# r-barnes/richdem

Hardware: AMD Instinct MI355X
Metric: Mcells/s Priority-Flood fill, 40k x 40k f32 DEM (higher is better)
Workload: dtype f32; 1 GPU; 40000x40000 float32 fractal value-noise DEM G(seed=3), FillDepressions<D8>, HBM-resident; cells=1600000000, basins=10332798, boruvka_rounds=9, pair_records=39443188, jump_passes=1, parallelism=1 GPU

## Files before the change

### richdem_amd/csrc/fill.hip

```cpp
#include "common.hpp"

#include <algorithm>
#include <cstdlib>
#include <vector>

struct rdgpu_fill_shard;

namespace rdgpu {

constexpr int TW = 64;
constexpr int TH = 32;
constexpr int LW = TW + 2;
constexpr int LH = TH + 2;
constexpr int NTHR = 256;
constexpr uint32_t OUTP = 0xFFFFFFFFu;
constexpr uint32_t CLOSED = 0x80000000u;
constexpr uint32_t NO_TID = 0xFFFFFFFFu;

static thread_local rdgpu_fill_stats g_stats;

constexpr int DW = 64, DH = 64, DLW = DW + 2, DLH = DH + 2;
constexpr uint32_t LAB_PEND = 0x80000000u;
constexpr uint16_t LTERM_BASE = 0xF000u;

// ... 2115 lines not shown
  const uint32_t n = st * rcap + i;
  const uint32_t c = cur[curN[n] & ~CLOSED] & ~CLOSED;
  nodeW[n] = c == B ? NO_TID : tid[c];
}

template <class T, int TOPO>
__global__ __launch_bounds__(NTHR) void k_shard_edges16(const T *__restrict__ z, const uint16_t *__restrict__ lab16,
                                                        const uint32_t *__restrict__ tile_base, uint32_t dtx,
                                                        const uint32_t *__restrict__ nodeW, const uint32_t *__restrict__ lvl,
                                                        int w, int h, unsigned long long *hkeys, uint32_t *hvals, uint32_t hmask,
                                                        uint32_t *overflow, uint32_t tilesX, uint32_t ntiles) {
  __shared__ uint32_t sl[ELH * ELW];
  __shared__ uint32_t sw[ELH * ELW];
  const uint32_t t = xcd_tile(blockIdx.x, ntiles);
  if (t >= ntiles) return;
  const int x0 = (int)(t % tilesX) * EW, y0 = (int)(t / tilesX) * EH;
  constexpr int IPT = (ELH * ELW + NTHR - 1) / NTHR;
  uint32_t nv[IPT], kv[IPT];
  bool ok[IPT];
#pragma unroll
  for (int r = 0; r < IPT; r++) {
    const int i = threadIdx.x + r * NTHR;
    const int ly = i / ELW, lx = i - ly * ELW;
    const int gx = x0 - 1 + lx, gy = y0 + ly;
    ok[r] = i < ELH * ELW && gx >= 0 && gx < w && gy < h;
    const int cx = ok[r] ? gx : 0, cy = ok[r] ? gy : 0;
    const size_t g = (size_t)cy * w + cx;
    nv[r] = tile_base[(uint32_t)(cy / DH) * dtx + (uint32_t)(cx / DW)] + lab16[g];
    kv[r] = Key32<T>::to(z[g]);
  }
  uint32_t wv[IPT], av[IPT];
#pragma unroll
  for (int r = 0; r < IPT; r++) {
    wv[r] = nodeW[nv[r]];
    av[r] = lvl[nv[r]];
  }
#pragma unroll
  for (int r = 0; r < IPT; r++) {
    const int i = threadIdx.x + r * NTHR;
    if (i < ELH * ELW) {
      sl[i] = ok[r] ? wv[r] : E_INVALID;
      sw[i] = av[r] > kv[r] ? av[r] : kv[r];
    }
  }
  __syncthreads();
  const int lx = threadIdx.x & (EW - 1), ly0 = threadIdx.x >> 6;
#pragma unroll 2
  for (int j = 0; j < EH / 4; j++) {
    const int ly = ly0 + 4 * j;
    const int o = ly * ELW + lx + 1;
    const uint32_t la = sl[o];
    if (la == E_INVALID) continue;
    const uint32_t wa = sw[o];
#pragma unroll
    for (int k = 0; k < 4; k++) {
      if (TOPO == 4 && (k == 1 || k == 3)) continue;
      const int q = o + (k == 0 ? 1 : k == 1 ? ELW - 1 : k == 2 ? ELW : ELW + 1);
      const uint32_t lb = sl[q];
      if (lb == la || lb == E_INVALID) continue;
      const uint32_t wb = sw[q];
      const uint32_t pass = wa > wb ? wa : wb;
      const uint32_t lo = la < lb ? la : lb, hi = la < lb ? lb : la;
      const unsigned long long key = (((unsigned long long)lo << 32) | hi) + 1ull;
      uint32_t slot = (uint32_t)((key * 0x9E3779B97F4A7C15ull) >> 32) & hmask;
      for (uint32_t probe = 0;; probe++) {
        if (probe > hmask) { *overflow = 1; break; }
        unsigned long long cur_k = __hip_atomic_load(&hkeys[slot], __ATOMIC_RELAXED, __HIP_MEMORY_SCOPE_AGENT);
        if (cur_k == 0) cur_k = atomicCAS(&hkeys[slot], 0ull, key);
        if (cur_k == 0 || cur_k == key) {
          if (__hip_atomic_load(&hvals[slot], __ATOMIC_RELAXED, __HIP_MEMORY_SCOPE_AGENT) > pass) atomicMin(&hvals[slot], pass);
          break;
        }
        slot = (slot + 1) & hmask;
      }
    }
  }
}

__global__ __launch_bounds__(NTHR) void k_node_levels(const uint32_t *__restrict__ curN, const uint32_t *__restrict__ acc,
                                                      const unsigned long long *__restrict__ counters, uint32_t rcap,
                                                      uint32_t *lvl) {
  const uint32_t st = blockIdx.y, i = blockIdx.x * NTHR + threadIdx.x;
  if (i >= (uint32_t)(counters[st * FSTRIDE] >> 32)) return;
  const uint32_t n = st * rcap + i;
  lvl[n] = acc[curN[n] & ~CLOSED];
}

template <class T, bool VEC>
__global__ __launch_bounds__(NTHR) void k_finalize16(T *z, const uint16_t *__restrict__ lab16, const uint32_t *__restrict__ lvl,
                                                     const uint32_t *__restrict__ tile_base, const uint32_t *__restrict__ tile_count,
                                                     int w, int h, uint32_t tilesX, uint32_t ntiles,
                                                     const uint8_t *__restrict__ skip = nullptr,
                                                     const uint32_t *__restrict__ tlist = nullptr,
                                                     const uint32_t *__restrict__ curN = nullptr,
                                                     const uint32_t *__restrict__ acc = nullptr) {
  __shared__ uint32_t sl[DH * DW];
  const uint32_t t = tlist ? tlist[blockIdx.x] : xcd_tile(blockIdx.x, ntiles);
  if (t >= ntiles) return;
  if (skip && skip[t]) return;
  const int x0 = (int)(t % tilesX) * DW, y0 = (int)(t / tilesX) * DH;
  const int qx = threadIdx.x & 15, ry = threadIdx.x >> 4;
  const int gx = x0 + 4 * qx;
  Quad<T> zqs[DH / 16];
  Quad<uint16_t> lqs[DH / 16];
#pragma unroll
  for (int r = 0; r < DH / 16; r++) {
    const int gy = y0 + ry + 16 * r;
    const bool in = gx < w && gy < h;
    const size_t g = in ? (size_t)gy * w + gx : 0;
    zqs[r] = load_quad<T, VEC>(z + (g - (in ? gx : 0)), in ? gx : 0, w, T());
    lqs[r] = load_quad<uint16_t, VEC>(lab16 + (g - (in ? gx : 0)), in ? gx : 0, w, (uint16_t)0);
  }
  const uint32_t base = tile_base[t], cnt = tile_count[t];
  if (curN) {
    for (uint32_t i = threadIdx.x; i < cnt; i += NTHR) sl[i] = acc[curN[base + i] & ~CLOSED];
  } else {
    for (uint32_t i = threadIdx.x; i < cnt; i += NTHR) sl[i] = lvl[base + i];
  }
  __syncthreads();
#pragma unroll
  for (int r = 0; r < DH / 16; r++) {
    const int gy = y0 + ry + 16 * r;
    if (gx >= w || gy >= h) continue;
    const size_t g = (size_t)gy * w + gx;
    Quad<T> zq = zqs[r];
    const Quad<uint16_t> lq = lqs[r];
    bool any = false;
#pragma unroll
    for (int e = 0; e < 4; e++) {
      if (gx + e >= w) continue;
      const uint32_t L = sl[lq.v[e] & (uint16_t)(DW * DH - 1)];
      if (L > Key32<T>::to(zq.v[e])) { zq.v[e] = Key32<T>::from(L); any = true; }
    }
    if (any) {
      if (VEC) {
        struct alignas(4 * sizeof(T)) AQ { T v[4]; };
        AQ a;
#pragma unroll
        for (int e = 0; e < 4; e++) a.v[e] = zq.v[e];
        *reinterpret_cast<AQ *>(z + g) = a;
      } else {
#pragma unroll
        for (int e = 0; e < 4; e++)
          if (gx + e < w) z[g + e] = zq.v[e];
      }
    }
  }
}

constexpr int NT_CAP = 1024;
static_assert(NT_CAP * 4 <= TW * TH * 2, "the node table lives in the boundary list's storage");
static_assert(TW == DW && DH % TH == 0, "a scan tile lies inside one descent tile");
constexpr uint32_t NO_TILE = 0xFFFFFFFFu;
constexpr int RING = 2 * LW + 2 * TH;

__device__ __forceinline__ void pair_spill_local(const EdgeOut &eo, unsigned long long *best, uint32_t seg, uint32_t *seg_fill,
                                                 uint32_t lo, uint32_t hi, uint32_t key) {
  const unsigned long long cl = ((unsigned long long)key << 32) | hi, ch = ((unsigned long long)key << 32) | lo;
  if (!(lo & CLOSED) && cl < best[lo]) atomicMin(&best[lo], cl);
  if (!(hi & CLOSED) && ch < best[hi]) atomicMin(&best[hi], ch);
  const uint32_t g = atomicAdd(seg_fill, 1u);
  if (g < eo.seglimit) {
    const size_t i = (size_t)seg * eo.segcap + g;
    eo.a[i] = lo; eo.b[i] = hi; eo.k[i] = key;
  } else {
    *eo.overflow = 1;
  }
}

template <class T, int TOPO, bool VEC>
__global__ __launch_bounds__(NTHR) void k_pairs16(const T *__restrict__ z, const uint16_t *__restrict__ lab16,
                                                  const uint32_t *__restrict__ curN, unsigned long long *best,
                                                  int w, int h, uint32_t B, uint32_t tilesX,
                                                  const uint32_t *__restrict__ tiles_in, uint32_t nwork,
                                                  EdgeOut eo,
                                                  const uint32_t *__restrict__ tile_base,
                                                  const uint32_t *__restrict__ tile_count, uint32_t dtx,
                                                  const uint8_t *__restrict__ skip,
                                                  const uint32_t *__restrict__ edgeK, const uint16_t *__restrict__ edgeS) {
  __shared__ __attribute__((aligned(8))) uint32_t sk[LH * LW];
  __shared__ uint32_t sc[LH * LW];
  __shared__ __attribute__((aligned(4))) uint16_t list[TW * TH];
  uint32_t *const ntab = reinterpret_cast<uint32_t *>(list);
  __shared__ unsigned long long pt_pair[PT_SLOTS];
  __shared__ uint32_t pt_key[PT_SLOTS];
  __shared__ uint32_t nlist, pt_n, pt_base, seg_fill;
  uint32_t *const tab_id = sk;
  unsigned long long *const tab_val = reinterpret_cast<unsigned long long *>(sk + SC_SLOTS);

  const uint32_t xcd = blockIdx.x & 7u, kstep = gridDim.x >> 3, per = (nwork + 7u) / 8u;
  const uint32_t seg = blockIdx.x;
  uint32_t it = blockIdx.x >> 3;
  auto next_tile = [&](uint32_t &i) -> uint32_t {
    while (i < per) {
      const uint32_t wi = xcd * per + i;
      if (wi >= nwork) break;
      const uint32_t t = tiles_in ? tiles_in[wi] : wi;
      if (!skip) return t;
      const int x0 = (int)(t % tilesX) * TW, y0 = (int)(t / tilesX) * TH;
      if (!skip[(uint32_t)(y0 / DH) * dtx + (uint32_t)(x0 / DW)]) return t;
      i += kstep;
    }
    i = per;
    return NO_TILE;
  };
  if (threadIdx.x == 0) seg_fill = 0;

  Quad<T> zq[2];
  Quad<uint16_t> lq[2];
  T rz = T();
  uint32_t rl = 0, rtb = 0, rc = 0, tbC = 0, cnt = 0, rkey = 0;
  uint32_t nt[NT_CAP / NTHR];
  auto ring_y = [](int tid) { const int rk = min(tid, RING - 1); return rk < LW ? 0 : rk < 2 * LW ? LH - 1 : (rk - 2 * LW < TH ? rk - 2 * LW + 1 : rk - 2 * LW - TH + 1); };
  auto ring_x = [](int tid) { const int rk = min(tid, RING - 1); return rk < LW ? rk : rk < 2 * LW ? rk - LW : (rk - 2 * LW < TH ? 0 : LW - 1); };

  auto load_a = [&](uint32_t t, int tid) {
    const int x0 = (int)(t % tilesX) * TW, y0 = (int)(t / tilesX) * TH;
    const uint32_t dC = (uint32_t)(y0 / DH) * dtx + (uint32_t)(x0 / DW);
    tbC = tile_base[dC];
    cnt = tile_count[dC];
    {
      const int rx = ring_x(tid), ry = ring_y(tid);
      const int gx = min(max(x0 - 1 + rx, 0), w - 1), gy = min(max(y0 - 1 + ry, 0), h - 1);
      const bool col = edgeK && ry >= 1 && ry <= TH && tid < RING;
      const uint32_t dtn = (uint32_t)(gy / DH) * dtx + (uint32_t)(gx / DW);
      const size_t e = ((size_t)dtn * 2 + (rx == 0 ? 1 : 0)) * DH + (uint32_t)(gy % DH);
      const size_t g = col ? (size_t)y0 * w + x0 : (size_t)gy * w + gx;
      rtb = tile_base[dtn];
      rl = col ? (uint32_t)edgeS[e] : (uint32_t)lab16[g];
      rkey = col ? edgeK[e] : 0u;
      rz = z[g];
    }
    const size_t tile0 = (size_t)y0 * w + x0;
    const char *zt = reinterpret_cast<const char *>(z + tile0), *lt = reinterpret_cast<const char *>(lab16 + tile0);
#pragma unroll
    for (int r = 0; r < 2; r++) {
      const int i = tid + r * NTHR;
      const int ly = i / (TW / 4), q = i - ly * (TW / 4);
      const int gx = x0 + 4 * q, gy = y0 + ly;
      const bool ok = gy < h && gx < w;
      if (VEC) {
        const uint32_t cell = ok ? (uint32_t)ly * (uint32_t)w + 4u * (uint32_t)q : 0u;
        struct alignas(4 * sizeof(T)) AZ { T v[4]; };
        struct alignas(8) AL { uint16_t v[4]; };
        const AL a = *reinterpret_cast<const AL *>(lt + cell * (uint32_t)sizeof(uint16_t));
        const AZ b = *reinterpret_cast<const AZ *>(zt + cell * (uint32_t)sizeof(T));
#pragma unroll
        for (int e = 0; e < 4; e++) { lq[r].v[e] = a.v[e]; zq[r].v[e] = b.v[e]; }
      } else {
        const size_t row = ok ? (size_t)gy * w : 0;
        lq[r] = load_quad<uint16_t, false>(lab16 + row, ok ? gx : 0, w, (uint16_t)0);
        zq[r] = load_quad<T, false>(z + row, ok ? gx : 0, w, T());
        if (!ok)
#pragma unroll
          for (int e = 0; e < 4; e++) lq[r].v[e] = 0;
      }
    }
  };
  auto load_b = [&](int tid) {
    const uint32_t nn = (cnt <= (uint32_t)NT_CAP && cnt) ? cnt : 1u;
#pragma unroll
    for (int k = 0; k < NT_CAP / NTHR; k++) {
      const uint32_t idx = (uint32_t)tid + k * NTHR;
      nt[k] = curN[tbC + min(idx, nn - 1u)];
    }
    rc = curN[rtb + rl];
  };

  uint32_t t = next_tile(it);
  if (t == NO_TILE) return;
  load_a(t, (int)threadIdx.x);
  load_b((int)threadIdx.x);
  constexpr int ROWS = TH / 4;
  for (;;) {
    int tid = (int)threadIdx.x;
    asm volatile("" : "+v"(tid));
    const int lx = tid & (TW - 1), band = __builtin_amdgcn_readfirstlane(tid >> 6), lane = tid & 63;
    const int rly = ring_y(tid), rlx = ring_x(tid);
    const bool isring = tid < RING;
    const int x0 = (int)(t % tilesX) * TW, y0 = (int)(t / tilesX) * TH;
    const bool tabled = cnt <= (uint32_t)NT_CAP;
#pragma unroll
    for (int k = 0; k < NT_CAP / NTHR; k++) ntab[tid + k * NTHR] = nt[k];
    pt_pair[tid] = ~0ull;
    pt_key[tid] = 0xFFFFFFFFu;
    static_assert(PT_SLOTS == NTHR, "one slot per thread");
    if (tid == 0) { nlist = 0; pt_n = 0; }
    __syncthreads();
    {
      uint32_t cq[2][4];
      if (tabled) {
#pragma unroll
        for (int r = 0; r < 2; r++)
#pragma unroll
          for (int e = 0; e < 4; e++) cq[r][e] = ntab[lq[r].v[e]];
      } else {
#pragma unroll
        for (int r = 0; r < 2; r++)
#pragma unroll
          for (int e = 0; e < 4; e++) cq[r][e] = curN[tbC + (uint32_t)lq[r].v[e]];
      }
      if (x0 + TW <= w && y0 + TH <= h) {
#pragma unroll
        for (int r = 0; r < 2; r++) {
          const int i = tid + r * NTHR;
          const int ly = i / (TW / 4), q = i - ly * (TW / 4);
          const int o = (ly + 1) * LW + 1 + 4 * q;
#pragma unroll
          for (int e = 0; e < 4; e++) {
            sk[o + e] = Key32<T>::to(zq[r].v[e]);
            sc[o + e] = cq[r][e];
          }
        }
      } else {
#pragma unroll
        for (int r = 0; r < 2; r++) {
          const int i = tid + r * NTHR;
          const int ly = i / (TW / 4), q = i - ly * (TW / 4);
          const int gx = x0 + 4 * q, gy = y0 + ly;
          const int o = (ly + 1) * LW + 1 + 4 * q;
#pragma unroll
          for (int e = 0; e < 4; e++) {
            const bool in = gy < h && gx + e < w;
            sk[o + e] = in ? Key32<T>::to(zq[r].v[e]) : 0u;
            sc[o + e] = in ? cq[r][e] : (B | CLOSED);
          }
        }
      }
      if (isring) {
        const int gx = x0 - 1 + rlx, gy = y0 - 1 + rly;
        const bool ok = gx >= 0 && gx < w && gy >= 0 && gy < h;
        const bool col = edgeK && rly >= 1 && rly <= TH;
        sk[rly * LW + rlx] = ok ? (col ? rkey : Key32<T>::to(rz)) : 0u;
        sc[rly * LW + rlx] = ok ? rc : (B | CLOSED);
      }
    }
    it += kstep;
    const uint32_t tn = next_tile(it);
    const uint32_t tl = tn != NO_TILE ? tn : t;
    load_a(tl, tid);
    __syncthreads();
    const int gxl = x0 + lx;
    const int yb = band * ROWS;
    {
      uint32_t c1[3], c2[3];
      {
        const int o = (yb + 1) * LW + lx;
#pragma unroll
        for (int e = 0; e < 3; e++) c1[e] = sc[o + e];
      }
      unsigned long long bal[ROWS];
      bool bnd[ROWS];
      const int rows_in = min(h - y0 - yb, ROWS);
      const bool colin = gxl < w;
#pragma unroll
      for (int j = 0; j < ROWS; j++) {
        const int ly = yb + j;
        {
          const int o = (ly + 2) * LW + lx;
#pragma unroll
          for (int e = 0; e < 3; e++) c2[e] = sc[o + e];
        }
        const uint32_t C = c1[1];
        uint32_t df = (c1[2] ^ C) | (c2[1] ^ C);
        if (TOPO == 8) df |= (c2[0] ^ C) | (c2[2] ^ C);
        bnd[j] = df != 0 && colin && j < rows_in;
        bal[j] = __builtin_amdgcn_ballot_w64(bnd[j]);
#pragma unroll
        for (int e = 0; e < 3; e++) c1[e] = c2[e];
      }
      uint32_t total = 0;
#pragma unroll
      for (int j = 0; j < ROWS; j++) total += (uint32_t)__popcll(bal[j]);
      if (total) {
        uint32_t base = 0;
        if (lane == 0) base = atomicAdd(&nlist, total);
        base = __shfl(base, 0, 64);
#pragma unroll
        for (int j = 0; j < ROWS; j++) {
          if (bnd[j])
            list[base + __builtin_amdgcn_mbcnt_hi((uint32_t)(bal[j] >> 32), __builtin_amdgcn_mbcnt_lo((uint32_t)bal[j], 0u))] =
                (uint16_t)((yb + j + 1) * LW + lx + 1);
          base += (uint32_t)__popcll(bal[j]);
        }
      }
    }
    __syncthreads();
    load_b(tid);
    const uint32_t nl = nlist;
    constexpr int NF = TOPO == 8 ? 4 : 2;
    const int foff[4] = {1, TOPO == 8 ? LW + 1 : LW, LW, LW - 1};
    for (uint32_t i = tid; i < nl; i += NTHR) {
      const int o = list[i];
      const uint32_t C = sc[o], kc = sk[o];
      uint32_t nD[NF], nH[NF];
#pragma unroll
      for (int e = 0; e < NF; e++) { nD[e] = sc[o + foff[e]]; nH[e] = sk[o + foff[e]]; }
      uint32_t pd[2] = {C, C}, pk[2] = {0xFFFFFFFFu, 0xFFFFFFFFu};
#pragma unroll
      for (int e = 0; e < NF; e++) {
        const uint32_t D = nD[e], hn = nH[e] > kc ? nH[e] : kc;
        if (D != C && !(C & D & CLOSED)) {
          if (pd[0] == C) pd[0] = D;
          if (D == pd[0]) pk[0] = hn < pk[0] ? hn : pk[0];
          else {
            if (pd[1] == C) pd[1] = D;
            if (D == pd[1]) pk[1] = hn < pk[1] ? hn : pk[1];
            else if (!pair_insert(pt_pair, pt_key, C < D ? C : D, C < D ? D : C, hn))
              pair_spill_local(eo, best, seg, &seg_fill, C < D ? C : D, C < D ? D : C, hn);
          }
        }
      }
      uint32_t ps[2], pq[2], lo[2], hi[2];
      unsigned long long pv[2];
#pragma unroll
      for (int j = 0; j < 2; j++) {
        lo[j] = C < pd[j] ? C : pd[j];
        hi[j] = C < pd[j] ? pd[j] : C;
        ps[j] = pair_home(lo[j], hi[j]);
        pv[j] = pt_pair[ps[j]];
        pq[j] = pt_key[ps[j]];
      }
#pragma unroll
      for (int j = 0; j < 2; j++) {
        if (pd[j] != C) {
          const unsigned long long pr = ((unsigned long long)lo[j] << 32) | hi[j];
          if (pv[j] == pr) { if (pk[j] < pq[j]) atomicMin(&pt_key[ps[j]], pk[j]); }
          else if (!pair_insert(pt_pair, pt_key, lo[j], hi[j], pk[j])) pair_spill_local(eo, best, seg, &seg_fill, lo[j], hi[j], pk[j]);
        }
      }
    }
    __syncthreads();
    tab_id[tid] = 0xFFFFFFFFu;
    tab_val[tid] = ~0ull;
    static_assert(SC_SLOTS == NTHR, "one slot per thread");
    {
      const bool occ = pt_pair[tid] != ~0ull;
      const unsigned long long bal = __ballot(occ);
      uint32_t base = 0;
      if (lane == 0 && bal) base = atomicAdd(&pt_n, (uint32_t)__popcll(bal));
      base = __shfl(base, 0, 64);
      if (occ) list[base + __popcll(bal & ((1ull << lane) - 1ull))] = (uint16_t)tid;
    }
    __syncthreads();
    const uint32_t tot = pt_n;
    if (tid == 0) {
      uint32_t ob = seg_fill;
      if (ob + tot > eo.seglimit) { *eo.overflow = 1; ob = 0xFFFFFFFFu; }
      else seg_fill = ob + tot;
      pt_base = ob;
    }
    for (uint32_t i = tid; i < tot; i += NTHR) {
      const int sl = list[i];
      const unsigned long long pr = pt_pair[sl];
      const uint32_t lo = (uint32_t)(pr >> 32), hi = (uint32_t)pr, key = pt_key[sl];
      if (!(lo & CLOSED)) {
        const unsigned long long cand = ((unsigned long long)key << 32) | hi;
        const int slot = tab_slot(tab_id, lo);
        if (slot >= 0) atomicMin(&tab_val[slot], cand);
        else if (cand < best[lo]) atomicMin(&best[lo], cand);
      }
      if (!(hi & CLOSED)) {
        const unsigned long long cand = ((unsigned long long)key << 32) | lo;
        const int slot = tab_slot(tab_id, hi);
        if (slot >= 0) atomicMin(&tab_val[slot], cand);
        else if (cand < best[hi]) atomicMin(&best[hi], cand);
      }
    }
    __syncthreads();
    {
      const uint32_t C = tab_id[tid];
      if (C != 0xFFFFFFFFu) {
        const unsigned long long cand = tab_val[tid];
        if (cand < best[C]) atomicMin(&best[C], cand);
      }
    }
    const uint32_t ob = pt_base;
    if (ob != 0xFFFFFFFFu) {
      const size_t g0 = (size_t)seg * eo.segcap + ob;
      for (uint32_t i = tid; i < tot; i += NTHR) {
        const int sl = list[i];
        const unsigned long long pr = pt_pair[sl];
        eo.a[g0 + i] = (uint32_t)(pr >> 32);
        eo.b[g0 + i] = (uint32_t)pr;
        eo.k[g0 + i] = pt_key[sl];
      }
    }
    __syncthreads();
    if (tn == NO_TILE) break;
    t = tn;
  }
  if (threadIdx.x == 0) eo.segcount[seg] = min(seg_fill, eo.seglimit);
}

template <class F>
static void with_flag(bool b, F &&f) {
  if (b) f(std::true_type());
  else f(std::false_type());
}

template <class T>
static void fill_finalize16(T *d_z, int w, int h, const FillBuffers &fb, hipStream_t s) {
  if (fb.trivial) return;
  const uint32_t dtx = cdiv(w, DW), dnt = dtx * cdiv(h, DH);
  const dim3 ngrid(cdiv(std::max(fb.nnmax, 1u), NTHR), fb.nstripes);
  RD_LAUNCH("fill.node_levels", k_node_levels, ngrid, dim3(NTHR), 0, s, (const uint32_t *)fb.curN, (const uint32_t *)fb.acc,
            (const unsigned long long *)fb.counters, fb.rcap, fb.lvl);
  const bool vec = (w % 4) == 0 && (reinterpret_cast<uintptr_t>(d_z) % (4 * sizeof(T))) == 0;
  with_flag(vec, [&](auto V) {
    RD_LAUNCH("fill.finalize", (k_finalize16<T, V>), dim3(xcd_grid(dnt)), dim3(NTHR), 0, s, d_z, (const uint16_t *)fb.lab16,
              (const uint32_t *)fb.lvl, (const uint32_t *)fb.tile_base, (const uint32_t *)fb.tile_count, w, h, dtx, dnt,
              (const uint8_t *)nullptr, (const uint32_t *)nullptr);
  });
}

template <class K>
static int pairs_blocks(K kernel) {
  int dev = 0, cus = 0, bpc = 0;
  RD_HIP(hipGetDevice(&dev));
  RD_HIP(hipDeviceGetAttribute(&cus, hipDeviceAttributeMultiprocessorCount, dev));
  RD_HIP(hipOccupancyMaxActiveBlocksPerMultiprocessor(&bpc, kernel, NTHR, 0));
  return std::max(8, (cus * std::max(bpc, 1)) / 8 * 8);
}

struct SparseLists {
  const uint32_t *d = nullptr;
  uint32_t stride = 0, n[3] = {0, 0, 0};
};
template <class T, int TOPO>
static bool fill_fused(T *d_z, int w, int h, hipStream_t s, const uint8_t *outlet = nullptr, const uint8_t *skip = nullptr,
                       const SparseLists *lists = nullptr, FillBuffers *keep = nullptr, BufAlloc *alloc = nullptr,
                       int open_top = 0, int open_bottom = 0) {
  const char *env_edges = getenv("RDGPU_FILL_EDGES");
  if (env_edges && env_edges[0] == '0') return false;
  const uint64_t n64 = (uint64_t)w * (uint64_t)h;
  if (n64 > 0x7FFF0000ull) throw Error(RDGPU_ERR_ARG, "rdgpu_fill: raster (or shard) has more than 2^31-65536 cells");
  const uint32_t n = (uint32_t)n64;
  if (w <= 2 || h <= 2) return false;
  g_stats = rdgpu_fill_stats{n64, 0, 0, 0, 0, (uint32_t)(TW * TH), 0};
  Workspace &ws = Workspace::get();
  uint32_t *hw = ws.host_words();
  const uint32_t dtx = cdiv(w, DW), dty = cdiv(h, DH), dnt = dtx * dty;
  const uint32_t tilesX = cdiv(w, TW), tilesY = cdiv(h, TH), ntiles = tilesX * tilesY;
  const bool vec = (w % 4) == 0 && (reinterpret_cast<uintptr_t>(d_z) % (4 * sizeof(T))) == 0;
  FusedBuf fo;
  fo.gcap = n / 4 + 4096;
  uint32_t nstripes = 1;
  while (nstripes < (uint32_t)FSTRIPES && fo.gcap / (2 * nstripes) >= 8192u && dnt >= 8 * nstripes) nstripes *= 2;
  fo.rcap = fo.gcap / nstripes;
  fo.smask = nstripes - 1;
  const bool sharded = keep != nullptr;
  if (sharded && !(open_top || open_bottom)) return false;
  auto persistent = [&](const char *name, size_t bytes) -> void * {
    return sharded ? (void *)alloc->get<uint8_t>(name, bytes) : ws.buf(name, bytes);
  };
  fo.lab16 = (uint16_t *)persistent("fused.lab16", (size_t)n * 2);
  fo.G = (uint32_t *)persistent("fused.G", (size_t)fo.gcap * 4);
  fo.tile_base = (uint32_t *)persistent("fused.tile_base", (size_t)dnt * 4);
  fo.tile_count = (uint32_t *)persistent("fused.tile_count", (size_t)dnt * 4);
  uint32_t *dflags = ws.buf<uint32_t>("fused.flags", 16);
  fo.counters = (unsigned long long *)persistent("fused.counters", (size_t)FSTRIPES * FSTRIDE * 8);
  uint32_t *pitoff = ws.buf<uint32_t>("fused.pitoff", FSTRIPES);
  fo.overflow = dflags + 5;
  uint32_t *curN = (uint32_t *)persistent("fused.curN", (size_t)fo.gcap * 4);
  if (!outlet) {
    fo.edgeK = ws.buf<uint32_t>("fused.edgeK", (size_t)dnt * 2 * DH);
    fo.edgeS = ws.buf<uint16_t>("fused.edgeS", (size_t)dnt * 2 * DH);
    fo.edgeR = ws.buf<uint16_t>("fused.edgeR", (size_t)dnt * 2 * DW);
  }
  RD_HIP(hipMemsetAsync(dflags, 0, 16 * sizeof(uint32_t), s));
  RD_HIP(hipMemsetAsync(fo.counters, 0, (size_t)FSTRIPES * FSTRIDE * sizeof(unsigned long long), s));
  if (outlet) {
    static const uint32_t one = 1u, outp = OUTP;
    RD_HIP(hipMemcpyAsync(reinterpret_cast<uint32_t *>(fo.counters) + 1, &one, sizeof(uint32_t), hipMemcpyHostToDevice, s));
    RD_HIP(hipMemcpyAsync(fo.G, &outp, sizeof(uint32_t), hipMemcpyHostToDevice, s));
  }
  const bool listed = outlet && skip && lists && lists->d;
  const uint32_t *dl = listed ? lists->d : nullptr, *sl_ = listed ? lists->d + lists->stride : nullptr,
                 *fl = listed ? lists->d + 2 * (size_t)lists->stride : nullptr;
  if (listed && lists->n[0] == 0) return true;
  with_flag(vec, [&](auto V) {
    auto descent = [&](auto OUTLETS, auto CUT) {
      RD_LAUNCH("fill.descent", (k_descent16<T, TOPO, V, OUTLETS, CUT>), dim3(listed ? lists->n[0] : xcd_grid(dnt)), dim3(NTHR), 0, s,
                (const T *)d_z, fo, w, h, dtx, dnt, outlet, skip, dl, open_top, open_bottom);
    };
    if (outlet) descent(std::true_type(), std::false_type());
    else if (sharded) descent(std::false_type(), std::true_type());
    else descent(std::false_type(), std::false_type());
  });
  RD_LAUNCH("fill.stripe_offsets", k_stripe_offsets, dim3(1), dim3(64), 0, s, (const unsigned long long *)fo.counters, nstripes, pitoff,
            dflags + 8);
  RD_HIP(hipMemcpyAsync(hw, dflags + 4, 8 * sizeof(uint32_t), hipMemcpyDeviceToHost, s));
  RD_HIP(hipStreamSynchronize(s));
  g_stats.host_syncs++;
  if (hw[1] != 0) { if (getenv("RDGPU_FILL_DEBUG")) fprintf(stderr, "fill_fused: node table overflow (nstripes %u rcap %u)\n", nstripes, fo.rcap); return false; }
  const uint32_t B = hw[4], NNmax = hw[6];
  g_stats.basins = B;
  if (sharded) {
    *keep = FillBuffers();
    keep->B = B;
    if (B == 0) { keep->trivial = true; return true; }
  }
  if (B == 0) return true;
  const dim3 ngrid(cdiv(std::max(NNmax, 1u), NTHR), nstripes);
  uint32_t *tid = nullptr;
  if (sharded) {
    tid = alloc->get<uint32_t>("fill.tid", (size_t)B + 1);
    RD_HIP(hipMemsetAsync(tid, 0xFF, ((size_t)B + 1) * sizeof(uint32_t), s));
    RD_LAUNCH("fill.mark_terminals", k_mark_terminals16, dim3(cdiv(w, NTHR)), dim3(NTHR), 0, s, (const uint16_t *)fo.lab16,
              (const uint32_t *)fo.tile_base, (const uint32_t *)fo.G, (const uint32_t *)pitoff, fo.rcap, tid, w, h, dtx, open_top,
              open_bottom);
  }
  RD_LAUNCH("fill.resolve_nodes", k_resolve_nodes, ngrid, dim3(NTHR), 0, s, fo.G, (const unsigned long long *)fo.counters,
            (const uint32_t *)pitoff, fo.rcap, (const uint16_t *)fo.lab16, (const uint32_t *)fo.tile_base, w, dtx, B, curN, dflags,
            (const uint32_t *)tid, (const uint16_t *)fo.edgeS, (const uint16_t *)fo.edgeR);
  g_stats.jump_passes = 1;
  uint32_t *cur = sharded ? alloc->get<uint32_t>("fill.cur", (size_t)B + 1) : ws.buf<uint32_t>("fill.cur", (size_t)B + 1);
  uint32_t *acc = sharded ? alloc->get<uint32_t>("fill.acc", (size_t)B + 1) : ws.buf<uint32_t>("fill.acc", (size_t)B + 1);
  unsigned long long *best = ws.buf<unsigned long long>("fill.best", (size_t)B + 1);
  unsigned long long *link = ws.buf<unsigned long long>("fill.link", (size_t)B + 1);
  uint32_t *rootsA = ws.buf<uint32_t>("fill.rootsA", B);
  uint32_t *rootsB = ws.buf<uint32_t>("fill.rootsB", B);
  RD_HIP(hipMemsetAsync(dflags + 2, 0, sizeof(uint32_t), s));
  RD_LAUNCH("fill.init_tables", k_init_tables, dim3(cdiv((uint64_t)B + 1, NTHR)), dim3(NTHR), 0, s, cur, acc, link, rootsA,
            dflags + 2, (const uint32_t *)tid, B);
  uint32_t nroots0 = B;
  if (sharded) {
    RD_HIP(hipMemcpyAsync(hw, dflags + 2, sizeof(uint32_t), hipMemcpyDeviceToHost, s));
    RD_HIP(hipStreamSynchronize(s));
    g_stats.host_syncs++;
    nroots0 = hw[0];
  }
  const uint32_t nwork1 = listed ? lists->n[1] : ntiles;
  static thread_local int pb_cache[2] = {0, 0};
  int &pb = pb_cache[vec ? 1 : 0];
  if (!pb) pb = vec ? pairs_blocks(k_pairs16<T, TOPO, true>) : pairs_blocks(k_pairs16<T, TOPO, false>);
  const uint32_t pgrid = std::max(8u, std::min<uint32_t>(xcd_grid(std::max(nwork1, 1u)), (uint32_t)pb));
  const uint32_t nseg = pgrid;
  const char *env_cap = getenv("RDGPU_FILL_EDGE_CAP");
  const uint64_t cap = env_cap ? strtoull(env_cap, nullptr, 10) : std::min<uint64_t>(12ull * B, n / 2) + 2048;
  const uint32_t segcap = cdiv(cdiv(cap, nseg), NTHR * EPT) * (NTHR * EPT);
  const size_t ecap = (size_t)nseg * segcap;
  uint32_t *elist[2] = {ws.buf<uint32_t>("fill.edges0", 3 * ecap), nullptr};
  size_t pcap[2] = {ecap, 0};
  uint32_t *segcount = ws.buf<uint32_t>("fill.segcount", nseg);
  RD_HIP(hipMemsetAsync(segcount, 0, nseg * sizeof(uint32_t), s));
  EdgeOut eo{elist[0], elist[0] + ecap, elist[0] + 2 * ecap, segcount, segcap, nseg - 1, dflags + 5};
  eo.seglimit = env_cap ? (uint32_t)std::min<uint64_t>(segcap, std::max<uint64_t>(1, cdiv(cap, nseg))) : segcap;
  int ein = 0;
  bool eseg = true;
  constexpr int MAXR = 48;
  uint32_t *rc = ws.buf<uint32_t>("fused.round_counts", 4 * (MAXR + 2));
  RD_HIP(hipMemsetAsync(rc, 0, 4 * (MAXR + 2) * sizeof(uint32_t), s));
  hw[220] = nroots0;
  RD_HIP(hipMemcpyAsync(rc + 4, hw + 220, sizeof(uint32_t), hipMemcpyHostToDevice, s));
  pcap[1] = ecap;
  elist[1] = ws.buf<uint32_t>("fill.edges1", 3 * pcap[1]);
  const uint32_t gcap = 2048;
  int rdone = 0;
  uint32_t rounds_run = 0;
  uint32_t troots = TAIL_ROOTS;
  if (const char *env_tail = getenv("RDGPU_FILL_TAIL_ROOTS")) troots = (uint32_t)std::min<unsigned long long>(strtoull(env_tail, nullptr, 10), 0xFFFFFFFFull);
  const uint32_t trecs = (uint32_t)std::min<unsigned long long>((unsigned long long)troots * TAIL_RECS_PER_ROOT, 0xFFFFFFFFull);
  uint32_t *const rootsP[2] = {rootsA, rootsB};
  auto enqueue_tail = [&](int rlo, int rhi, int rmax) {
    TailArgs ta;
    ta.roots[0] = rootsP[0]; ta.roots[1] = rootsP[1];
    ta.el[0] = elist[0]; ta.el[1] = elist[1];
    ta.pcap = ecap; ta.segcount = segcount; ta.segcap = segcap;
    ta.cur = cur; ta.best = best; ta.link = link; ta.B = B; ta.rc = rc; ta.flag = dflags;
    ta.troots = troots; ta.trecs = trecs;
    ta.rlo = std::max(2, rlo); ta.rhi = rhi; ta.rmax = rmax; ta.maxhops = 1 << 14;
    RD_LAUNCH("fill.rounds_tail", k_rounds_tail, dim3(1), dim3(TAILT), 0, s, ta);
  };
  auto enqueue_round = [&](int r) {
    uint32_t *rootsA = rootsP[(r - 1) & 1], *rootsB = rootsP[r & 1];
    TailGate gate;
    if (troots && r >= 2) { gate.cnt = rc + 4 * r; gate.roots = troots; gate.recs = trecs; }
    const uint32_t bound = std::max(1u, r - 1 < 31 ? nroots0 >> (r - 1) : 1u);
    const uint32_t rgrid = std::min(gcap, cdiv(bound, NTHR));
    const uint32_t *nr = rc + 4 * r, *ne = rc + 4 * r + 1;
    uint32_t *nr_next = rc + 4 * (r + 1), *ne_next = rc + 4 * (r + 1) + 1;
    RD_LAUNCH("fill.best_reset", k_best_reset, dim3(rgrid), dim3(NTHR), 0, s, (const uint32_t *)rootsA, 0u, best, nr, gate);
    if (r == 1) {
      const uint32_t nwork = listed ? lists->n[1] : ntiles;
      if (nwork > 0)
        with_flag(vec, [&](auto V) {
          RD_LAUNCH("fill.scan", (k_pairs16<T, TOPO, V>), dim3(pgrid), dim3(NTHR), 0, s, (const T *)d_z, (const uint16_t *)fo.lab16,
                    (const uint32_t *)curN, best, w, h, B, tilesX, sl_, nwork, eo, (const uint32_t *)fo.tile_base,
                    (const uint32_t *)fo.tile_count, dtx, skip, (const uint32_t *)fo.edgeK, (const uint16_t *)fo.edgeS);
        });
      RD_LAUNCH("fill.sum_segments", k_sum_segments, dim3(1), dim3(NTHR), 0, s, (const uint32_t *)eo.segcount, nseg, rc + 4 * 1 + 1,
                rc + 4 * 2 + 1);
      g_stats.scan_tiles += ntiles;
    } else {
      const int eout = ein ^ 1;
      const uint32_t *ia = elist[ein], *ib = elist[ein] + pcap[ein], *ik = elist[ein] + 2 * pcap[ein];
      uint32_t *oa = elist[eout], *ob = elist[eout] + pcap[eout], *ok = elist[eout] + 2 * pcap[eout];
      if (eseg)
        RD_LAUNCH("fill.edge_round", (k_edge_round<true>), dim3(std::min<uint32_t>(4 * gcap, cdiv(ecap, NTHR * EPT))), dim3(NTHR), 0,
                  s, ia, ib, ik, (uint32_t)ecap, (const uint32_t *)segcount, segcap, (const uint32_t *)cur, best, B, oa, ob, ok, ne_next,
                  (const uint32_t *)nullptr, gate);
      else
        RD_LAUNCH("fill.edge_round", (k_edge_round<false>), dim3(gcap), dim3(NTHR), 0, s, ia, ib, ik, 0u,
                  (const uint32_t *)nullptr, 0u, (const uint32_t *)cur, best, B, oa, ob, ok, ne_next, ne, gate);
      eseg = false;
      ein = eout;
    }
    RD_LAUNCH("fill.hook", k_hook, dim3(rgrid), dim3(NTHR), 0, s, (const uint32_t *)rootsA, 0u, (const unsigned long long *)best, link, nr,
              gate);
    RD_LAUNCH("fill.chase_links", k_chase_links, dim3(rgrid), dim3(NTHR), 0, s, (const uint32_t *)rootsA, 0u, link, 1 << 14, dflags,
              nr, gate);
    RD_LAUNCH("fill.compact_roots", k_compact_roots, dim3(std::min(gcap, cdiv(bound, NTHR * RPT))), dim3(NTHR), 0, s,
              (const uint32_t *)rootsA, 0u, (const unsigned long long *)link, rootsB, nr_next, nr, cur, gate);
  };
  uint32_t *hrc = ws.host_words() + 16;
  {
    uint32_t lg = 0;
    while ((1ull << lg) < (unsigned long long)nroots0 + 1ull) lg++;
    int batch = std::min(MAXR, std::max(4, (int)(2 * lg + 4) / 5 + 1));
    if (troots) {
      int r4 = 2;
      while (r4 < batch && (2 * (r4 - 1) < 32 ? nroots0 >> (2 * (r4 - 1)) : 0u) > troots) r4++;
      batch = std::min(batch, r4);
    }
    const char *env_batch = getenv("RDGPU_FILL_ROUND_BATCH");
    if (env_batch) batch = std::min(MAXR, std::max(1, atoi(env_batch)));
    uint32_t last_live = 0xFFFFFFFFu;
    for (;;) {
      const int rfirst = rdone + 1;
      for (int k = 0; k < batch && rdone < MAXR; k++) enqueue_round(++rdone);
      if (troots) enqueue_tail(rfirst, env_batch ? rdone : std::min(rdone + 1, MAXR), env_batch ? rdone : MAXR);
      RD_HIP(hipMemcpyAsync(hrc, rc, 4 * (MAXR + 2) * sizeof(uint32_t), hipMemcpyDeviceToHost, s));
      RD_HIP(hipMemcpyAsync(hw, dflags, 14 * sizeof(uint32_t), hipMemcpyDeviceToHost, s));
      RD_HIP(hipStreamSynchronize(s));
      g_stats.host_syncs++;
      if (getenv("RDGPU_FILL_DEBUG")) fprintf(stderr, "fill_fused: pair pass: %u records, overflow %u, %u tiles on the slow road; %d rounds enqueued\n", hrc[4 + 1], hw[5], hw[12], rdone);
      if (hw[0] != 0) { if (getenv("RDGPU_FILL_DEBUG")) fprintf(stderr, "fill_fused: hook chain unfinished\n"); return false; }
      if (hw[5] != 0) { if (getenv("RDGPU_FILL_DEBUG")) fprintf(stderr, "fill_fused: pair list overflow (B %u cap %llu nseg %u segcap %u nwork %u)\n", B, (unsigned long long)cap, nseg, segcap, nwork1); return false; }
      if ((int)hrc[2] > rdone) rdone = std::min<int>(hrc[2], MAXR);
      rounds_run = 0;
      for (int r = 1; r <= rdone; r++) rounds_run += hrc[4 * r] != 0;
      g_stats.edge_records = hrc[4 + 1];
      const uint32_t live = hrc[4 * (rdone + 1)];
      if (live == 0) break;
      if (live >= last_live || rdone >= MAXR) throw Error(RDGPU_ERR_HIP, "rdgpu_fill: contraction made no progress (internal error)");
      last_live = live;
      if (!env_batch) batch = 4;
    }
  }
  g_stats.rounds += rounds_run;
  RD_LAUNCH("fill.settle_basins", k_settle_basins, dim3(cdiv(B, NTHR)), dim3(NTHR), 0, s, cur, acc, link, B, 1 << 14, dflags);
  if (sharded) {
    uint32_t *lvl = fo.G;
    RD_LAUNCH("fill.node_levels", k_node_levels, ngrid, dim3(NTHR), 0, s, (const uint32_t *)curN, (const uint32_t *)acc,
              (const unsigned long long *)fo.counters, fo.rcap, lvl);
    uint32_t *nodeW = alloc->get<uint32_t>("fused.nodeW", fo.gcap);
    RD_LAUNCH("fill.node_watersheds", k_node_watersheds, ngrid, dim3(NTHR), 0, s, (const uint32_t *)curN, (const uint32_t *)cur,
              (const uint32_t *)tid, (const unsigned long long *)fo.counters, fo.rcap, B, nodeW);
    keep->compact = true;
    keep->cur = cur; keep->acc = acc; keep->tid = tid;
    keep->lab16 = fo.lab16; keep->tile_base = fo.tile_base; keep->tile_count = fo.tile_count;
    keep->curN = curN; keep->lvl = lvl; keep->nodeW = nodeW; keep->counters = fo.counters;
    keep->rcap = fo.rcap; keep->nstripes = nstripes; keep->nnmax = NNmax;
    return true;
  }
  if (listed && lists->n[2] == 0) return true;
  with_flag(vec, [&](auto V) {
    RD_LAUNCH("fill.finalize", (k_finalize16<T, V>), dim3(listed ? lists->n[2] : xcd_grid(dnt)), dim3(NTHR), 0, s, d_z,
              (const uint16_t *)fo.lab16, (const uint32_t *)nullptr, (const uint32_t *)fo.tile_base, (const uint32_t *)fo.tile_count, w,
              h, dtx, dnt, skip, fl, (const uint32_t *)curN, (const uint32_t *)acc);
  });
  return true;
}

template <class T>
static void fill_device(T *d_z, int w, int h, int topology, hipStream_t s) {
  check_fill_args(d_z, w, h, topology);
  if (topology == 8 ? fill_fused<T, 8>(d_z, w, h, s) : fill_fused<T, 4>(d_z, w, h, s)) return;
  FillBuffers fb;
  BufAlloc ws_alloc{false, nullptr};
  if (topology == 8) fill_local_phase<T, 8>(d_z, w, h, 0, 0, ws_alloc, fb, s);
  else fill_local_phase<T, 4>(d_z, w, h, 0, 0, ws_alloc, fb, s);
  fill_finalize<T>(d_z, w, h, fb, s);
}

template <class T>
static void fill_outlets_device(T *d_z, const uint8_t *d_outlet, const uint8_t *d_skip, int w, int h, hipStream_t s,
                                const SparseLists *lists = nullptr) {
  check_fill_args(d_z, w, h, 8);
  if (!d_outlet) throw Error(RDGPU_ERR_ARG, "rdgpu_fill_outlets: null outlet mask");
  if (w <= 2 || h <= 2) return;
  if (fill_fused<T, 8>(d_z, w, h, s, d_outlet, d_skip, lists)) return;
  FillBuffers fb;
  BufAlloc ws_alloc{false, nullptr};
  fill_local_phase<T, 8>(d_z, w, h, 0, 0, ws_alloc, fb, s, d_outlet);
  fill_finalize<T>(d_z, w, h, fb, s);
}

template <class T>
static void fill_host(T *dem, int w, int h, int topology) {
  check_fill_args(dem, w, h, topology);
  const size_t bytes = (size_t)w * h * sizeof(T);
  T *d = Workspace::get().buf<T>("host.dem", (size_t)w * h);
  RD_HIP(hipMemcpy(d, dem, bytes, hipMemcpyHostToDevice));
  fill_device<T>(d, w, h, topology, nullptr);
  RD_HIP(hipStreamSynchronize(nullptr));
  RD_HIP(hipMemcpy(dem, d, bytes, hipMemcpyDeviceToHost));
}

}

struct rdgpu_fill_shard {
  int dtype = 0;
  void *d_dem = nullptr;
  int w = 0, h = 0, topology = 8, open_top = 0, open_bottom = 0;
  hipStream_t stream = nullptr;
  rdgpu::FillBuffers fb;
  std::vector<void *> owned;
  bool cached = false;
  int device = 0;
  uint32_t *d_edges = nullptr;
  uint32_t nedges = 0;
  rdgpu_fill_stats stats{};
};

namespace rdgpu {

template <class T>
struct DtypeCode;
template <> struct DtypeCode<uint8_t> { static constexpr int v = 0; };
template <> struct DtypeCode<int16_t> { static constexpr int v = 1; };
template <> struct DtypeCode<uint16_t> { static constexpr int v = 2; };
template <> struct DtypeCode<int32_t> { static constexpr int v = 3; };
template <> struct DtypeCode<uint32_t> { static constexpr int v = 4; };
template <> struct DtypeCode<float> { static constexpr int v = 5; };
template <> struct DtypeCode<int8_t> { static constexpr int v = 6; };

// ... 474 lines not shown
```

Baseline: 106,300 Mcells/s.

## Pair scan tiles per descent tile and share halo, node table and spill

The scan kernel now walks the two vertically stacked scan tiles of each 64x64 descent tile back to back in the unlisted path. The pair table reset and the edge flush happen only once per pair, and the node table is reloaded only for the first tile. The halo is reduced to a one-sided ring (bottom row plus left and right columns), and shared tiles use a padded 16-byte-aligned layout so interior cells are written with uint4 stores. Work count and segment capacity are switched to descent tiles, which changes load balance across blocks and edge-buffer sizing.

```diff
diff --git a/richdem_amd/csrc/fill.hip b/richdem_amd/csrc/fill.hip
--- a/richdem_amd/csrc/fill.hip
+++ b/richdem_amd/csrc/fill.hip
@@ -2291,7 +2291,10 @@
 static_assert(NT_CAP * 4 <= TW * TH * 2, "the node table lives in the boundary list's storage");
 static_assert(TW == DW && DH % TH == 0, "a scan tile lies inside one descent tile");
 constexpr uint32_t NO_TILE = 0xFFFFFFFFu;
-constexpr int RING = 2 * LW + 2 * TH;
+constexpr int PLW = TW + 8, PX = 4, PLH = TH + 1;
+constexpr int RING = LW + 2 * TH;
+static_assert((PLW % 4) == 0 && (PX % 4) == 0, "quads of a row are 16-byte aligned");
+static_assert(PLH * PLW < 65536 && PLH * PLW * 4 >= SC_SLOTS * 12, "list entries are 16-bit offsets; the component table fits the keys' storage");
 
 __device__ __forceinline__ void pair_spill_local(const EdgeOut &eo, unsigned long long *best, uint32_t seg, uint32_t *seg_fill,
                                                  uint32_t lo, uint32_t hi, uint32_t key) {
@@ -2317,8 +2320,8 @@
                                                   const uint32_t *__restrict__ tile_count, uint32_t dtx,
                                                   const uint8_t *__restrict__ skip,
                                                   const uint32_t *__restrict__ edgeK, const uint16_t *__restrict__ edgeS) {
-  __shared__ __attribute__((aligned(8))) uint32_t sk[LH * LW];
-  __shared__ uint32_t sc[LH * LW];
+  __shared__ __attribute__((aligned(16))) uint32_t sk[PLH * PLW];
+  __shared__ __attribute__((aligned(16))) uint32_t sc[PLH * PLW];
   __shared__ __attribute__((aligned(4))) uint16_t list[TW * TH];
   uint32_t *const ntab = reinterpret_cast<uint32_t *>(list);
   __shared__ unsigned long long pt_pair[PT_SLOTS];
@@ -2330,14 +2333,24 @@
   const uint32_t xcd = blockIdx.x & 7u, kstep = gridDim.x >> 3, per = (nwork + 7u) / 8u;
   const uint32_t seg = blockIdx.x;
   uint32_t it = blockIdx.x >> 3;
-  auto next_tile = [&](uint32_t &i) -> uint32_t {
+  const bool paired = tiles_in == nullptr;
+  auto next_tile = [&](uint32_t &i, uint32_t &m) -> uint32_t {
+    m = 0;
     while (i < per) {
       const uint32_t wi = xcd * per + i;
       if (wi >= nwork) break;
-      const uint32_t t = tiles_in ? tiles_in[wi] : wi;
-      if (!skip) return t;
-      const int x0 = (int)(t % tilesX) * TW, y0 = (int)(t / tilesX) * TH;
-      if (!skip[(uint32_t)(y0 / DH) * dtx + (uint32_t)(x0 / DW)]) return t;
+      if (paired) {
+        if (!skip || !skip[wi]) {
+          const uint32_t dy = wi / dtx;
+          m = (int)(2 * dy + 1) * TH < h ? 1u : 0u;
+          return wi + dy * tilesX;
+        }
+      } else {
+        const uint32_t t = tiles_in[wi];
+        if (!skip) return t;
+        const int x0 = (int)(t % tilesX) * TW, y0 = (int)(t / tilesX) * TH;
+        if (!skip[(uint32_t)(y0 / DH) * dtx + (uint32_t)(x0 / DW)]) return t;
+      }
       i += kstep;
     }
     i = per;
@@ -2350,8 +2363,8 @@
   T rz = T();
   uint32_t rl = 0, rtb = 0, rc = 0, tbC = 0, cnt = 0, rkey = 0;
   uint32_t nt[NT_CAP / NTHR];
-  auto ring_y = [](int tid) { const int rk = min(tid, RING - 1); return rk < LW ? 0 : rk < 2 * LW ? LH - 1 : (rk - 2 * LW < TH ? rk - 2 * LW + 1 : rk - 2 * LW - TH + 1); };
-  auto ring_x = [](int tid) { const int rk = min(tid, RING - 1); return rk < LW ? rk : rk < 2 * LW ? rk - LW : (rk - 2 * LW < TH ? 0 : LW - 1); };
+  auto ring_y = [](int tid) { const int rk = min(tid, RING - 1); return rk < LW ? TH : (rk - LW < TH ? rk - LW : rk - LW - TH); };
+  auto ring_x = [](int tid) { const int rk = min(tid, RING - 1); return rk < LW ? rk - 1 : (rk - LW < TH ? -1 : TW); };
 
   auto load_a = [&](uint32_t t, int tid) {
     const int x0 = (int)(t % tilesX) * TW, y0 = (int)(t / tilesX) * TH;
@@ -2360,10 +2373,10 @@
     cnt = tile_count[dC];
     {
       const int rx = ring_x(tid), ry = ring_y(tid);
-      const int gx = min(max(x0 - 1 + rx, 0), w - 1), gy = min(max(y0 - 1 + ry, 0), h - 1);
-      const bool col = edgeK && ry >= 1 && ry <= TH && tid < RING;
+      const int gx = min(max(x0 + rx, 0), w - 1), gy = min(max(y0 + ry, 0), h - 1);
+      const bool col = edgeK && ry < TH && tid < RING;
       const uint32_t dtn = (uint32_t)(gy / DH) * dtx + (uint32_t)(gx / DW);
-      const size_t e = ((size_t)dtn * 2 + (rx == 0 ? 1 : 0)) * DH + (uint32_t)(gy % DH);
+      const size_t e = ((size_t)dtn * 2 + (rx < 0 ? 1 : 0)) * DH + (uint32_t)(gy % DH);
       const size_t g = col ? (size_t)y0 * w + x0 : (size_t)gy * w + gx;
       rtb = tile_base[dtn];
       rl = col ? (uint32_t)edgeS[e] : (uint32_t)lab16[g];
@@ -2396,20 +2409,25 @@
       }
     }
   };
-  auto load_b = [&](int tid) {
-    const uint32_t nn = (cnt <= (uint32_t)NT_CAP && cnt) ? cnt : 1u;
-#pragma unroll
-    for (int k = 0; k < NT_CAP / NTHR; k++) {
-      const uint32_t idx = (uint32_t)tid + k * NTHR;
-      nt[k] = curN[tbC + min(idx, nn - 1u)];
+  auto load_b = [&](int tid, bool newtab) {
+    if (newtab) {
+      if (cnt <= (uint32_t)NTHR) {
+        nt[0] = curN[tbC + min((uint32_t)tid, max(cnt, 1u) - 1u)];
+      } else if (cnt <= (uint32_t)NT_CAP) {
+#pragma unroll
+        for (int k = 0; k < NT_CAP / NTHR; k++) nt[k] = curN[tbC + min((uint32_t)tid + k * NTHR, cnt - 1u)];
+      }
     }
     rc = curN[rtb + rl];
   };
 
-  uint32_t t = next_tile(it);
+  uint32_t mode = 0;
+  uint32_t t = next_tile(it, mode);
   if (t == NO_TILE) return;
+#pragma unroll
+  for (int k = 0; k < NT_CAP / NTHR; k++) nt[k] = 0;
   load_a(t, (int)threadIdx.x);
-  load_b((int)threadIdx.x);
+  load_b((int)threadIdx.x, true);
   constexpr int ROWS = TH / 4;
   for (;;) {
     int tid = (int)threadIdx.x;
@@ -2419,10 +2437,17 @@
     const bool isring = tid < RING;
     const int x0 = (int)(t % tilesX) * TW, y0 = (int)(t / tilesX) * TH;
     const bool tabled = cnt <= (uint32_t)NT_CAP;
-#pragma unroll
-    for (int k = 0; k < NT_CAP / NTHR; k++) ntab[tid + k * NTHR] = nt[k];
-    pt_pair[tid] = ~0ull;
-    pt_key[tid] = 0xFFFFFFFFu;
+    const bool first = mode != 2u, last = mode != 1u;
+    if (cnt <= (uint32_t)NTHR) {
+      ntab[tid] = nt[0];
+    } else if (tabled) {
+#pragma unroll
+      for (int k = 0; k < NT_CAP / NTHR; k++) ntab[tid + k * NTHR] = nt[k];
+    }
+    if (first) {
+      pt_pair[tid] = ~0ull;
+      pt_key[tid] = 0xFFFFFFFFu;
+    }
     static_assert(PT_SLOTS == NTHR, "one slot per thread");
     if (tid == 0) { nlist = 0; pt_n = 0; }
     __syncthreads();
@@ -2444,12 +2469,9 @@
         for (int r = 0; r < 2; r++) {
           const int i = tid + r * NTHR;
           const int ly = i / (TW / 4), q = i - ly * (TW / 4);
-          const int o = (ly + 1) * LW + 1 + 4 * q;
-#pragma unroll
-          for (int e = 0; e < 4; e++) {
-            sk[o + e] = Key32<T>::to(zq[r].v[e]);
-            sc[o + e] = cq[r][e];
-          }
+          const int o = ly * PLW + PX + 4 * q;
+          *reinterpret_cast<uint4 *>(sk + o) = make_uint4(Key32<T>::to(zq[r].v[0]), Key32<T>::to(zq[r].v[1]), Key32<T>::to(zq[r].v[2]), Key32<T>::to(zq[r].v[3]));
+          *reinterpret_cast<uint4 *>(sc + o) = make_uint4(cq[r][0], cq[r][1], cq[r][2], cq[r][3]);
         }
       } else {
 #pragma unroll
@@ -2457,25 +2479,29 @@
           const int i = tid + r * NTHR;
           const int ly = i / (TW / 4), q = i - ly * (TW / 4);
           const int gx = x0 + 4 * q, gy = y0 + ly;
-          const int o = (ly + 1) * LW + 1 + 4 * q;
+          const int o = ly * PLW + PX + 4 * q;
+          uint32_t kq[4];
 #pragma unroll
           for (int e = 0; e < 4; e++) {
             const bool in = gy < h && gx + e < w;
-            sk[o + e] = in ? Key32<T>::to(zq[r].v[e]) : 0u;
-            sc[o + e] = in ? cq[r][e] : (B | CLOSED);
+            kq[e] = in ? Key32<T>::to(zq[r].v[e]) : 0u;
+            cq[r][e] = in ? cq[r][e] : (B | CLOSED);
           }
+          *reinterpret_cast<uint4 *>(sk + o) = make_uint4(kq[0], kq[1], kq[2], kq[3]);
+          *reinterpret_cast<uint4 *>(sc + o) = make_uint4(cq[r][0], cq[r][1], cq[r][2], cq[r][3]);
         }
       }
       if (isring) {
-        const int gx = x0 - 1 + rlx, gy = y0 - 1 + rly;
+        const int gx = x0 + rlx, gy = y0 + rly;
         const bool ok = gx >= 0 && gx < w && gy >= 0 && gy < h;
-        const bool col = edgeK && rly >= 1 && rly <= TH;
-        sk[rly * LW + rlx] = ok ? (col ? rkey : Key32<T>::to(rz)) : 0u;
-        sc[rly * LW + rlx] = ok ? rc : (B | CLOSED);
-      }
-    }
-    it += kstep;
-    const uint32_t tn = next_tile(it);
+        const bool col = edgeK && rly < TH;
+        sk[rly * PLW + PX + rlx] = ok ? (col ? rkey : Key32<T>::to(rz)) : 0u;
+        sc[rly * PLW + PX + rlx] = ok ? rc : (B | CLOSED);
+      }
+    }
+    uint32_t tn, mn = 2u;
+    if (mode == 1u) tn = t + tilesX;
+    else { it += kstep; tn = next_tile(it, mn); }
     const uint32_t tl = tn != NO_TILE ? tn : t;
     load_a(tl, tid);
     __syncthreads();
@@ -2484,7 +2510,7 @@
     {
       uint32_t c1[3], c2[3];
       {
-        const int o = (yb + 1) * LW + lx;
+        const int o = yb * PLW + PX - 1 + lx;
 #pragma unroll
         for (int e = 0; e < 3; e++) c1[e] = sc[o + e];
       }
@@ -2496,7 +2522,7 @@
       for (int j = 0; j < ROWS; j++) {
         const int ly = yb + j;
         {
-          const int o = (ly + 2) * LW + lx;
+          const int o = (ly + 1) * PLW + PX - 1 + lx;
 #pragma unroll
           for (int e = 0; e < 3; e++) c2[e] = sc[o + e];
         }
@@ -2519,16 +2545,16 @@
         for (int j = 0; j < ROWS; j++) {
           if (bnd[j])
             list[base + __builtin_amdgcn_mbcnt_hi((uint32_t)(bal[j] >> 32), __builtin_amdgcn_mbcnt_lo((uint32_t)bal[j], 0u))] =
-                (uint16_t)((yb + j + 1) * LW + lx + 1);
+                (uint16_t)((yb + j) * PLW + PX + lx);
           base += (uint32_t)__popcll(bal[j]);
         }
       }
     }
     __syncthreads();
-    load_b(tid);
+    load_b(tid, mode != 1u);
     const uint32_t nl = nlist;
     constexpr int NF = TOPO == 8 ? 4 : 2;
-    const int foff[4] = {1, TOPO == 8 ? LW + 1 : LW, LW, LW - 1};
+    const int foff[4] = {1, TOPO == 8 ? PLW + 1 : PLW, PLW, PLW - 1};
     for (uint32_t i = tid; i < nl; i += NTHR) {
       const int o = list[i];
       const uint32_t C = sc[o], kc = sk[o];
@@ -2570,64 +2596,67 @@
       }
     }
     __syncthreads();
-    tab_id[tid] = 0xFFFFFFFFu;
-    tab_val[tid] = ~0ull;
-    static_assert(SC_SLOTS == NTHR, "one slot per thread");
-    {
-      const bool occ = pt_pair[tid] != ~0ull;
-      const unsigned long long bal = __ballot(occ);
-      uint32_t base = 0;
-      if (lane == 0 && bal) base = atomicAdd(&pt_n, (uint32_t)__popcll(bal));
-      base = __shfl(base, 0, 64);
-      if (occ) list[base + __popcll(bal & ((1ull << lane) - 1ull))] = (uint16_t)tid;
-    }
-    __syncthreads();
-    const uint32_t tot = pt_n;
-    if (tid == 0) {
-      uint32_t ob = seg_fill;
-      if (ob + tot > eo.seglimit) { *eo.overflow = 1; ob = 0xFFFFFFFFu; }
-      else seg_fill = ob + tot;
-      pt_base = ob;
-    }
-    for (uint32_t i = tid; i < tot; i += NTHR) {
-      const int sl = list[i];
-      const unsigned long long pr = pt_pair[sl];
-      const uint32_t lo = (uint32_t)(pr >> 32), hi = (uint32_t)pr, key = pt_key[sl];
-      if (!(lo & CLOSED)) {
-        const unsigned long long cand = ((unsigned long long)key << 32) | hi;
-        const int slot = tab_slot(tab_id, lo);
-        if (slot >= 0) atomicMin(&tab_val[slot], cand);
-        else if (cand < best[lo]) atomicMin(&best[lo], cand);
-      }
-      if (!(hi & CLOSED)) {
-        const unsigned long long cand = ((unsigned long long)key << 32) | lo;
-        const int slot = tab_slot(tab_id, hi);
-        if (slot >= 0) atomicMin(&tab_val[slot], cand);
-        else if (cand < best[hi]) atomicMin(&best[hi], cand);
-      }
-    }
-    __syncthreads();
-    {
-      const uint32_t C = tab_id[tid];
-      if (C != 0xFFFFFFFFu) {
-        const unsigned long long cand = tab_val[tid];
-        if (cand < best[C]) atomicMin(&best[C], cand);
-      }
-    }
-    const uint32_t ob = pt_base;
-    if (ob != 0xFFFFFFFFu) {
-      const size_t g0 = (size_t)seg * eo.segcap + ob;
+    if (last) {
+      tab_id[tid] = 0xFFFFFFFFu;
+      tab_val[tid] = ~0ull;
+      static_assert(SC_SLOTS == NTHR, "one slot per thread");
+      {
+        const bool occ = pt_pair[tid] != ~0ull;
+        const unsigned long long bal = __ballot(occ);
+        uint32_t base = 0;
+        if (lane == 0 && bal) base = atomicAdd(&pt_n, (uint32_t)__popcll(bal));
+        base = __shfl(base, 0, 64);
+        if (occ) list[base + __popcll(bal & ((1ull << lane) - 1ull))] = (uint16_t)tid;
+      }
+      __syncthreads();
+      const uint32_t tot = pt_n;
+      if (tid == 0) {
+        uint32_t ob = seg_fill;
+        if (ob + tot > eo.seglimit) { *eo.overflow = 1; ob = 0xFFFFFFFFu; }
+        else seg_fill = ob + tot;
+        pt_base = ob;
+      }
       for (uint32_t i = tid; i < tot; i += NTHR) {
         const int sl = list[i];
         const unsigned long long pr = pt_pair[sl];
-        eo.a[g0 + i] = (uint32_t)(pr >> 32);
-        eo.b[g0 + i] = (uint32_t)pr;
-        eo.k[g0 + i] = pt_key[sl];
-      }
-    }
-    __syncthreads();
+        const uint32_t lo = (uint32_t)(pr >> 32), hi = (uint32_t)pr, key = pt_key[sl];
+        if (!(lo & CLOSED)) {
+          const unsigned long long cand = ((unsigned long long)key << 32) | hi;
+          const int slot = tab_slot(tab_id, lo);
+          if (slot >= 0) atomicMin(&tab_val[slot], cand);
+          else if (cand < best[lo]) atomicMin(&best[lo], cand);
+        }
+        if (!(hi & CLOSED)) {
+          const unsigned long long cand = ((unsigned long long)key << 32) | lo;
+          const int slot = tab_slot(tab_id, hi);
+          if (slot >= 0) atomicMin(&tab_val[slot], cand);
+          else if (cand < best[hi]) atomicMin(&best[hi], cand);
+        }
+      }
+      __syncthreads();
+      {
+        const uint32_t C = tab_id[tid];
+        if (C != 0xFFFFFFFFu) {
+          const unsigned long long cand = tab_val[tid];
+          if (cand < best[C]) atomicMin(&best[C], cand);
+        }
+      }
+      const uint32_t ob = pt_base;
+      if (ob != 0xFFFFFFFFu) {
+        const size_t g0 = (size_t)seg * eo.segcap + ob;
+        for (uint32_t i = tid; i < tot; i += NTHR) {
+          const int sl = list[i];
+          const unsigned long long pr = pt_pair[sl];
+          eo.a[g0 + i] = (uint32_t)(pr >> 32);
+          eo.b[g0 + i] = (uint32_t)pr;
+          eo.k[g0 + i] = pt_key[sl];
+        }
+      }
+      __syncthreads();
+    }
     if (tn == NO_TILE) break;
     t = tn;
+    mode = mn;
   }
   if (threadIdx.x == 0) eo.segcount[seg] = min(seg_fill, eo.seglimit);
 }
@@ -2770,7 +2799,7 @@
     g_stats.host_syncs++;
     nroots0 = hw[0];
   }
-  const uint32_t nwork1 = listed ? lists->n[1] : ntiles;
+  const uint32_t nwork1 = listed ? lists->n[1] : dnt;
   static thread_local int pb_cache[2] = {0, 0};
   int &pb = pb_cache[vec ? 1 : 0];
   if (!pb) pb = vec ? pairs_blocks(k_pairs16<T, TOPO, true>) : pairs_blocks(k_pairs16<T, TOPO, false>);
@@ -2778,7 +2807,7 @@
   const uint32_t nseg = pgrid;
   const char *env_cap = getenv("RDGPU_FILL_EDGE_CAP");
   const uint64_t cap = env_cap ? strtoull(env_cap, nullptr, 10) : std::min<uint64_t>(12ull * B, n / 2) + 2048;
-  const uint32_t segcap = cdiv(cdiv(cap, nseg), NTHR * EPT) * (NTHR * EPT);
+  const uint32_t segcap = std::max<uint32_t>(cdiv(cdiv(cap, std::min(nseg, std::max(nwork1, 1u))), NTHR * EPT), 4u) * (NTHR * EPT);
   const size_t ecap = (size_t)nseg * segcap;
   uint32_t *elist[2] = {ws.buf<uint32_t>("fill.edges0", 3 * ecap), nullptr};
   size_t pcap[2] = {ecap, 0};
@@ -2822,7 +2851,7 @@
     uint32_t *nr_next = rc + 4 * (r + 1), *ne_next = rc + 4 * (r + 1) + 1;
     RD_LAUNCH("fill.best_reset", k_best_reset, dim3(rgrid), dim3(NTHR), 0, s, (const uint32_t *)rootsA, 0u, best, nr, gate);
     if (r == 1) {
-      const uint32_t nwork = listed ? lists->n[1] : ntiles;
+      const uint32_t nwork = nwork1;
       if (nwork > 0)
         with_flag(vec, [&](auto V) {
           RD_LAUNCH("fill.scan", (k_pairs16<T, TOPO, V>), dim3(pgrid), dim3(NTHR), 0, s, (const T *)d_z, (const uint16_t *)fo.lab16,
```

Result: slower. 103,600 Mcells/s (-2.5%).
